# taaha-khan/2023-CompaCT-Image-Compression

Measured on AMD Instinct MI355X. Metric: MPixels/s encode+decode, 12-bit 512x512 CT batch, bytes-exact, higher is better.
Workload: dtype u16

## Files before the change

2023-compact-image-compression_amd/csrc/api.cpp:

```cpp
#include <dlfcn.h>
#include <unistd.h>
#include <zlib.h>

#include <atomic>
#include <chrono>
#include <condition_variable>
#include <functional>
#include <cstdarg>
#include <cstdio>
#include <cstdlib>
#include <cstring>
#include <map>
#include <mutex>
#include <string>
#include <thread>
#include <vector>

#include "../../include/compact_hip.h"
#include "cct_internal.h"
#include "host.h"

namespace cct {
bool gilbert_table(int width, int height, int32_t *out);

// ... 31 lines not shown
	std::mutex *mu = nullptr;
	hipStream_t stream = nullptr;
	struct ZGraph { std::vector<uint8_t> key; hipGraph_t graph = nullptr; hipGraphExec_t exec = nullptr; uint64_t last_use = 0; };
	std::vector<ZGraph> z_graphs;
	uint64_t z_clock = 0;
	hipStream_t stream_copy = nullptr;
	hipEvent_t ev_pack[2] = {nullptr, nullptr}, ev_copied[2] = {nullptr, nullptr};
	DevBuf z_packed2[2];
	unsigned pack_slot = 0;
	DevBuf e_role, e_lidx, e_lmask, e_lcur, e_images, e_payload, e_sizes, e_status, e_stats;
	DevBuf e_pairrec, e_hand;
	DevBuf h_stage;
	DevBuf h_small[2];
	DevBuf z_vals_in, z_vals_out, z_mr, z_rec, z_exitp, z_exitc, z_sym, z_bentry, z_bsym,
	    z_small, z_bend, z_meta, z_tables, z_sorttmp, z_out, z_outsizes, z_in, z_insizes, z_packed, z_packoffs, z_gen, z_runs;
	const void *z_mr_cleared = nullptr;
	size_t z_mr_cleared_cap = 0;
	unsigned z_gen_passes = 0;
	hipEvent_t ev_k0s[2] = {nullptr, nullptr}, ev_k1s[2] = {nullptr, nullptr};
	hipEvent_t ev_z0s[2] = {nullptr, nullptr}, ev_z1s[2] = {nullptr, nullptr};
	hipEvent_t ev_small[2] = {nullptr, nullptr};
	hipStream_t stream_side = nullptr;
	hipEvent_t ev_fork[4] = {nullptr, nullptr, nullptr, nullptr};
	unsigned call_parity = 0;
	DevBuf *all_bufs[48];
	int n_bufs = 0;
	EncSlot()
	{
		DevBuf *b[] = {&e_role, &e_lidx, &e_lmask, &e_lcur, &e_images, &e_payload, &e_sizes, &e_status, &e_stats, &e_pairrec,
		               &e_hand, &h_stage, &z_vals_in, &z_vals_out, &z_mr, &z_rec, &z_exitp, &z_exitc,
		               &z_sym, &z_bentry, &z_bsym, &z_small, &z_bend, &z_meta, &z_tables, &z_sorttmp, &z_out, &z_outsizes, &z_in,
		               &z_insizes, &z_packed, &z_packoffs, &z_packed2[0], &z_packed2[1], &z_gen, &z_runs, &h_small[0], &h_small[1]};
// ... 549 lines not shown
		ta.e = a;
		ta.tile_org = tb->d_org; ta.tile_orient = tb->d_orient; ta.patterns = tb->d_pat;
		ta.n_orient = tb->n_orient; ta.n_tiles = tb->n_tiles; ta.row_pitch = width;
		HIP_TRY(launch_encode_tiles(ta, n, st));
		g_ctx.last_path = 2;
		return CCT_OK;
	}
	const bool run_time = bs_run_time(bs, g_ctx.runtime_bs != 0);
	HIP_TRY(launch_encode(a, n, bs, g_ctx.wg_threads, st, run_time));
	g_ctx.last_path = run_time ? 4 : 0;
	return CCT_OK;
}

constexpr size_t DEFLATE_PASS_BYTES = (size_t)1 << 30;

int deflate_locked(EncSlot &E, const uint8_t *d_in, size_t in_stride, const uint32_t *d_in_sizes, int n, const uint8_t header13[13],
                   size_t out_stride, int level, int strategy)
{
	if (in_stride % 256 != 0 || out_stride % 4 != 0) return fail(CCT_E_ARG, "deflate strides must be multiples of 256 / 4");
	DeflateArgs a{};
	if (!deflate_strategy_args(level, strategy, a))
		return fail(CCT_E_ARG, "zlib level %d with strategy %d is not on the device", level, strategy);
	const bool chains = strategy != 2 && strategy != 3, walk = strategy != 2;
	const size_t EB = (size_t)n * in_stride;
	if (EB >= ((size_t)1 << 32)) return fail(CCT_E_ARG, "deflate batch of %zu bytes exceeds the 4 GiB sort limit; split the batch", EB);
	const int max_blocks = (int)(in_stride / 16383 + 2);
	int rc;
	if (chains) {
		if ((rc = E.z_vals_in.ensure(EB * 8))) return rc;
		if ((rc = E.z_vals_out.ensure(EB * 8))) return rc;
// ... 3 lines not shown
	}
	if ((rc = E.z_sym.ensure(EB * 4))) return rc;
	if (walk) {
		if ((rc = E.z_exitp.ensure(EB * 4))) return rc;
		if ((rc = E.z_exitc.ensure(EB * 4))) return rc;
		if ((rc = E.z_bentry.ensure(EB / 64 * 4))) return rc;
		if ((rc = E.z_bsym.ensure(EB / 64 * 4))) return rc;
	}
	const int run_chunks = (int)(in_stride / 1784 + 1);
	if ((rc = E.z_small.ensure((size_t)n * (9 + 384 + 2 * (size_t)run_chunks) * 4))) return rc;
	if ((rc = E.z_bend.ensure((size_t)n * max_blocks * 4))) return rc;
	if ((rc = E.z_meta.ensure((size_t)n * max_blocks * sizeof(BlockMeta)))) return rc;
	if ((rc = E.z_tables.ensure((size_t)n * max_blocks * sizeof(BlockTables)))) return rc;
	if ((rc = E.z_out.ensure((size_t)n * out_stride))) return rc;
	if ((rc = E.z_outsizes.ensure((size_t)n * 4))) return rc;
	const size_t tmp = (deflate_sort_temp_bytes((size_t)n * in_stride, n) + 511) & ~(size_t)255;
	if ((rc = E.z_sorttmp.ensure(tmp + 256))) return rc;
	const bool use_fork = g_ctx.deflate_fork != 0;
	if (use_fork && !E.stream_side) {
		const int crc = exclusive_section([&]() -> int { HIP_TRY(hipStreamCreateWithFlags(&E.stream_side, hipStreamNonBlocking)); return CCT_OK; });
		if (crc) return crc;
	}
	a.in = d_in; a.in_stride = in_stride; a.in_sizes = d_in_sizes;
	a.rec_in = (uint64_t *)E.z_vals_in.p; a.rec_out = (uint64_t *)E.z_vals_out.p;
	a.pos_mask = (g_ctx.compact_recs && in_stride < ((size_t)1 << 22)) ? (1u << 22) - 1u : 0xFFFFFFFFu;
	uint32_t *small = (uint32_t *)E.z_small.p;
	a.seg_begin = small; a.seg_end = small + n; a.total_syms = small + 2 * n; a.postloop_lit = small + 3 * n;
	a.n_blocks = small + 4 * n; a.adler = small + 5 * n; a.heavy_count = small + 6 * n; a.deep_count = small + 7 * n; a.run_end_count = small + 8 * n; a.sort_hist = small + 9 * n;
	a.run_counts = small + (9 + 384) * (size_t)n; a.run_chunks = run_chunks;
	if ((rc = E.z_gen.ensure(256))) return rc;
	if (chains && (E.z_mr_cleared != E.z_mr.p || E.z_mr_cleared_cap != E.z_mr.cap || E.z_gen_passes >= 16000u)) {
		HIP_TRY(hipMemsetAsync(E.z_mr.p, 0, E.z_mr.cap, E.stream));
		HIP_TRY(hipMemsetAsync(E.z_gen.p, 0, 256, E.stream));
		E.z_mr_cleared = E.z_mr.p; E.z_mr_cleared_cap = E.z_mr.cap; E.z_gen_passes = 0;
	}
	if (chains) E.z_gen_passes++;
	a.gen = (uint32_t *)E.z_gen.p;
	a.mr = E.z_mr.p; a.heavy_list = (uint32_t *)E.z_rec.p; a.sym = (uint32_t *)E.z_sym.p;
	a.run_ends = (uint32_t *)E.z_runs.p;
	a.run_len = (uint16_t *)E.z_sym.p;
	a.rec32 = (uint32_t *)E.z_exitp.p; a.exit_pos = (uint32_t *)E.z_exitc.p; a.exit_cnt = (uint32_t *)E.z_rec.p;
	a.blk_entry = (uint32_t *)E.z_bentry.p; a.blk_symbase = (uint32_t *)E.z_bsym.p;
	a.blk_end = (uint32_t *)E.z_bend.p;
	a.block_meta = (BlockMeta *)E.z_meta.p; a.block_tables = (BlockTables *)E.z_tables.p;
	a.max_blocks = max_blocks;
	a.out = (uint8_t *)E.z_out.p; a.out_stride = out_stride; a.out_sizes = (uint32_t *)E.z_outsizes.p;
	memcpy(a.header13, header13, 13);
	if (g_ctx.use_graph) {
		std::vector<uint8_t> key(sizeof(DeflateArgs) + 2 * sizeof(int));
		memcpy(key.data(), &a, sizeof(DeflateArgs));
		memcpy(key.data() + sizeof(DeflateArgs), &n, sizeof(int));
		const int fork_key = use_fork ? 1 : 0;
		memcpy(key.data() + sizeof(DeflateArgs) + sizeof(int), &fork_key, sizeof(int));
		EncSlot::ZGraph *zg = nullptr;
		for (auto &g : E.z_graphs) if (g.key == key) zg = &g;
		if (!zg) {
			const int crc = exclusive_section([&]() -> int {
				if (E.z_graphs.size() >= 4) {
					size_t old = 0;
					for (size_t i = 1; i < E.z_graphs.size(); i++) if (E.z_graphs[i].last_use < E.z_graphs[old].last_use) old = i;
					if (E.z_graphs[old].exec) (void)hipGraphExecDestroy(E.z_graphs[old].exec);
					if (E.z_graphs[old].graph) (void)hipGraphDestroy(E.z_graphs[old].graph);
					E.z_graphs.erase(E.z_graphs.begin() + (long)old);
				}
				EncSlot::ZGraph g;
				HIP_TRY(hipStreamBeginCapture(E.stream, hipStreamCaptureModeThreadLocal));
				hipError_t le = launch_deflate(a, n, E.z_sorttmp.p, tmp, E.stream, use_fork ? E.stream_side : nullptr, E.ev_fork);
				hipError_t ce = hipStreamEndCapture(E.stream, &g.graph);
				if (le != hipSuccess) { if (g.graph) (void)hipGraphDestroy(g.graph); return fail(CCT_E_DEVICE, "DEFLATE capture: %s", hipGetErrorString(le)); }
				HIP_TRY(ce);
				const hipError_t ie = hipGraphInstantiate(&g.exec, g.graph, nullptr, nullptr, 0);
				if (ie != hipSuccess) { (void)hipGraphDestroy(g.graph); return fail(CCT_E_DEVICE, "hipGraphInstantiate failed: %s", hipGetErrorString(ie)); }
				g.key = key;
				E.z_graphs.push_back(std::move(g));
				return CCT_OK;
			});
			if (crc) return crc;
			zg = &E.z_graphs.back();
		}
		zg->last_use = ++E.z_clock;
		HIP_TRY(hipGraphLaunch(zg->exec, E.stream));
		return CCT_OK;
	}
	HIP_TRY(launch_deflate(a, n, E.z_sorttmp.p, tmp, E.stream, use_fork ? E.stream_side : nullptr, E.ev_fork));
	return CCT_OK;
}

int decode_payload_locked(DecSlot &D, const uint8_t *d_payload, size_t stride, const uint32_t *d_sizes, int n, int width,
                          int height, int bs, int fractal, uint16_t *d_images, uint32_t *d_status, hipStream_t st)
{
	const int N = width * height, NB = N / bs;
	if (stride % 16 != 0) return fail(CCT_E_ARG, "payload stride must be a multiple of 16");
	if (n == 0) return CCT_OK;
	DecArgs a{};
	a.payload = d_payload; a.stride = stride; a.sizes = d_sizes;
	a.lut = nullptr;
	a.n_tiles = 0; a.n_orient = 0; a.width = width;
	if (fractal) {
		const ShapeTables *tb;
// ... 565 lines not shown
				int e = -1; unsigned slot = 0;
				void release() { if (e >= 0) { { std::lock_guard<std::mutex> pl(g_pack_mu); g_pack_busy[e][slot] = false; } g_pack_cv.notify_all(); e = -1; } }
				~PackOwner() { release(); }
			} pack_owner;
			const bool queue_ahead = qa;
			if (queue_ahead) {
				HIP_TRY(hipEventRecord(E.ev_small[par], E.stream));
				{ std::lock_guard<std::mutex> pl(g_pack_mu); g_pack_busy[&E - g_enc][packed_slot] = true; }
				pack_owner.e = (int)(&E - g_enc); pack_owner.slot = (unsigned)packed_slot;
				lk.unlock();
				HIP_TRY(hipEventSynchronize(E.ev_small[par]));
				memcpy(psz.data(), l_psz, (size_t)n * 4); memcpy(h_status, l_status, (size_t)n * 4); memcpy(osz, l_osz, (size_t)nc * 4);
				if (h_stats) memcpy(h_stats, l_stats, (size_t)n * sizeof(cct_slice_stats));
			} else HIP_TRY(hipStreamSynchronize(E.stream));
			drain.disarm();
			HIP_TRY(hipEventElapsedTime(&t_dev_deflate_ms, ev_z0, ev_z1));
			if (one_pass) {
				HIP_TRY(hipEventElapsedTime(&tl_enc_kernel_ms, ev_k0, ev_k1));
				for (int i = 0; i < n; i++)
					if (h_status[i] & CCT_ST_CAP) return fail(CCT_E_CAP, "slice %d overflowed its payload stride", i);
			}
			tl_deflate_ms += t_dev_deflate_ms;
			const double t_c0 = now_ms();
			FilesOut f{E, nc, osz, zstride, 0, std::vector<size_t>(nc + 1, 0)};
			for (int i = 0; i < nc; i++) { f.exact += osz[i]; f.offs[i + 1] = f.offs[i] + (((size_t)osz[i] + 15) & ~(size_t)15); }
			if (packed_slot < 0 && (rc = E.z_packoffs.ensure((size_t)(nc + 1) * 8))) return rc;
			if (!packed) {
				if ((rc = files_to_strided(f, h_out + (size_t)c0 * out_stride, out_stride))) return rc;
				tl_d2h_ms += (float)(now_ms() - t_c0);
				continue;
// ... 85 lines not shown
	HIP_TRY(hipMemcpyAsync(E.z_insizes.p, isz.data(), (size_t)n * 4, hipMemcpyHostToDevice, E.stream));
	uint8_t hdr13[13] = {0};
	struct Events {
		hipEvent_t e[2] = {nullptr, nullptr};
		~Events() { for (hipEvent_t x : e) if (x) (void)hipEventDestroy(x); }
	} ev;
	HIP_TRY(hipEventCreate(&ev.e[0]));
	HIP_TRY(hipEventCreate(&ev.e[1]));
	HIP_TRY(hipEventRecord(ev.e[0], E.stream));
	rc = deflate_locked(E, (const uint8_t *)E.z_in.p, in_stride, (const uint32_t *)E.z_insizes.p, n, hdr13, zstride, level, strategy);
	if (rc) return rc;
	HIP_TRY(hipEventRecord(ev.e[1], E.stream));
	HIP_TRY(hipMemcpyAsync(osz.data(), E.z_outsizes.p, (size_t)n * 4, hipMemcpyDeviceToHost, E.stream));
	HIP_TRY(hipStreamSynchronize(E.stream));
	HIP_TRY(hipEventElapsedTime(&tl_deflate_ms, ev.e[0], ev.e[1]));
	for (int i = 0; i < n; i++) {
		h_out_sizes[i] = osz[i] - 13;
		HIP_TRY(hipMemcpyAsync(h_out + (size_t)i * out_stride, (uint8_t *)E.z_out.p + (size_t)i * zstride + 13, osz[i] - 13,
		                       hipMemcpyDeviceToHost, E.stream));
	}
	HIP_TRY(hipStreamSynchronize(E.stream));
	return CCT_OK;
}

int cct_zlib_compress_batch(const uint8_t *h_in, const uint64_t *h_offsets, int n, uint8_t *h_out, size_t out_stride,
                            uint32_t *h_out_sizes)
{
	return zlib_compress_batch_impl(h_in, h_offsets, n, 9, Z_DEFAULT_STRATEGY, h_out, out_stride, h_out_sizes);
}

// ... 326 lines not shown
```

2023-compact-image-compression_amd/csrc/cct_internal.h:

```cpp
#pragma once
#include <stddef.h>
#include <stdint.h>

#include <hip/hip_runtime.h>

namespace cct {

constexpr int ENC_CH = 8192;
constexpr int ENC_RING = 4;
constexpr int ENC_LIST_CAP = 1536;
constexpr int ENC_STG_BYTES = 2 * ENC_CH + ENC_CH / 8 + 64;
constexpr int ENC_MAX_LDS_ROLE = 48 * 1024;

constexpr uint8_t ROLE_PARTNER = 0xFF;

struct EncArgs {
	const uint16_t *images;
	const int32_t *lut;
	int N, NB;
	int eof;
	uint32_t flags;
	uint8_t *payload; size_t stride;
	uint32_t *sizes; uint32_t *status;
	uint8_t *ws_role;
// ... 92 lines not shown
struct BlockTables {
	uint16_t lcode[286]; uint8_t llen[286];
	uint16_t dcode[30]; uint8_t dlen[30];
	uint32_t hdr_bits[160];
};
struct DeflateArgs {
	const uint8_t *in; size_t in_stride; const uint32_t *in_sizes;
	uint64_t *rec_in, *rec_out;
	uint32_t pos_mask;
	uint32_t *seg_begin, *seg_end;
	void *mr;
	uint32_t *gen;
	uint32_t *heavy_list, *sym, *run_ends;
	uint32_t *run_counts; int run_chunks;
	uint32_t *sort_hist;
	uint16_t *run_len;
	uint32_t *rec32, *exit_pos, *exit_cnt;
	uint32_t *blk_entry, *blk_symbase;
	uint32_t *total_syms, *postloop_lit, *n_blocks, *adler, *heavy_count, *deep_count, *run_end_count;
	uint32_t *blk_end;
	BlockMeta *block_meta; BlockTables *block_tables;
	int max_blocks;
	uint8_t *out; size_t out_stride; uint32_t *out_sizes;
	uint8_t header13[16];
	uint32_t good, max_lazy, nice, max_chain, zlib_flg;
	uint32_t strategy, min_len;
};
bool deflate_level_args(int level, DeflateArgs &a);
bool deflate_strategy_args(int level, int strategy, DeflateArgs &a);
hipError_t deflate_init_tables();
size_t deflate_sort_temp_bytes(size_t total, int n);
hipError_t launch_pack(const uint8_t *src, size_t stride, const uint32_t *sizes, int n, uint64_t *offsets, uint8_t *dst,
                       int exact, hipStream_t st);
hipError_t launch_deflate(const DeflateArgs &a, int n, void *sort_temp, size_t sort_temp_bytes, hipStream_t st, hipStream_t side = nullptr,
                          const hipEvent_t *fork_join_events = nullptr);

hipError_t launch_gate_bump(uint32_t *word, hipStream_t st);
hipError_t launch_gate_wait(const uint32_t *gate, uint32_t want_pass, uint32_t grace_us, uint32_t timeout_us, hipStream_t st);

struct InflateArgs {
	const uint8_t *in; uint64_t in_total;
	const uint64_t *offsets; int skip;
	uint8_t *out; size_t out_stride;
	uint32_t *out_sizes, *status;
};
hipError_t launch_inflate(const InflateArgs &a, int n, hipStream_t st, int lanes);

hipError_t launch_packbits_encode(const uint8_t *d_in, const uint64_t *d_offsets, int n, int delta, uint32_t *d_ws, uint8_t *d_out,
                                  size_t out_stride, uint32_t *d_out_sizes, hipStream_t st);
// ... 5 lines not shown
```

2023-compact-image-compression_amd/csrc/deflate_kernels.hip:

```cpp
#include <hip/hip_runtime.h>
#include <cstring>
#include <algorithm>

#include "cct_internal.h"
#include "../../include/compact_hip.h"

namespace cct {
namespace {

constexpr int MIN_MATCH = 3, MAX_MATCH = 258, WSIZE = 32768;
constexpr int MIN_LOOKAHEAD = MAX_MATCH + MIN_MATCH + 1;
constexpr int MAX_DIST = WSIZE - MIN_LOOKAHEAD;
constexpr int TOO_FAR = 4096;
constexpr int BLOCK_SYMS = 16383;
constexpr int L_CODES = 286, D_CODES = 30, BL_CODES = 19, HEAP_SIZE = 2 * L_CODES + 1;
constexpr int END_BLOCK = 256, MAX_BITS = 15, MAX_BL_BITS = 7;
constexpr uint32_t Z_FILTERED = 1, Z_HUFFMAN_ONLY = 2, Z_RLE = 3, Z_FIXED = 4;
__host__ __device__ __forceinline__ bool short_pass(uint32_t strategy) { return strategy == Z_HUFFMAN_ONLY || strategy == Z_RLE; }

__constant__ uint8_t c_extra_lbits[29] = {0,0,0,0,0,0,0,0,1,1,1,1,2,2,2,2,3,3,3,3,4,4,4,4,5,5,5,5,0};
__constant__ uint8_t c_extra_dbits[30] = {0,0,0,0,1,1,2,2,3,3,4,4,5,5,6,6,7,7,8,8,9,9,10,10,11,11,12,12,13,13};
__constant__ uint8_t c_extra_blbits[19] = {0,0,0,0,0,0,0,0,0,0,0,0,0,0,0,0,2,3,7};
__constant__ uint8_t c_bl_order[19] = {16,17,18,0,8,7,9,6,10,5,11,4,12,3,13,2,14,1,15};
__constant__ uint8_t c_length_code[256];
// ... 27 lines not shown
	return o;
}

__device__ __forceinline__ void lds_barrier()
{
	asm volatile("s_waitcnt lgkmcnt(0)\n\ts_barrier" ::: "memory");
}

__device__ __forceinline__ uint32_t wave_sum(uint32_t v)
{
#pragma unroll
	for (int d = 32; d >= 1; d >>= 1) v += (uint32_t)__shfl_xor((int)v, d, 64);
	return v;
}

template <bool FIRST>
__global__ void __launch_bounds__(1024) dfl_sort_pass_kernel(DeflateArgs a)
{
	constexpr int BITS = FIRST ? 8 : 7, NB = 1 << BITS;
	__shared__ uint32_t offs[256];
	__shared__ uint32_t wcnt[16][NB];
	const int s = blockIdx.x;
	const uint32_t L = a.in_sizes[s];
	const uint8_t *in = a.in + (size_t)s * a.in_stride;
	const size_t base = (size_t)s * a.in_stride;
	const uint32_t npos = L >= MIN_MATCH ? L - 2 : 0;
	const uint64_t *rec_src = a.rec_in + base;
	uint64_t *rec_dst = (FIRST ? a.rec_in : a.rec_out) + base;
	const int tid = threadIdx.x, lane = tid & 63, wave = tid >> 6;
	const uint64_t lt_mask = (1ull << lane) - 1ull;
	if (tid < 256) offs[tid] = 0;
	__syncthreads();
	if (tid < NB) offs[tid] = a.sort_hist[(size_t)s * 384 + (FIRST ? 0 : 256) + tid];
	__syncthreads();
	if (wave == 0) {
		uint32_t v[4], sum = 0;
#pragma unroll
		for (int k = 0; k < 4; k++) { v[k] = offs[lane * 4 + k]; sum += v[k]; }
		uint32_t inc = sum;
#pragma unroll
		for (int d = 1; d < 64; d <<= 1) { const uint32_t o = (uint32_t)__shfl_up((int)inc, d, 64); if (lane >= d) inc += o; }
		uint32_t run = inc - sum;
#pragma unroll
		for (int k = 0; k < 4; k++) { offs[lane * 4 + k] = run; run += v[k]; }
	}
	__syncthreads();
#ifndef CCT_SORT_E
#define CCT_SORT_E 4
#endif
	constexpr int E = CCT_SORT_E;
	constexpr int ND = E / 4;
	const uint32_t last = npos ? npos - 1 : 0;
	static_assert(E % 4 == 0 && ND + 1 <= E, "pass A: whole dwords per lane, kept in ra[0 .. ND]");
#ifdef CCT_SORT_PROBE
	const bool compact = false;
#else
	const bool compact = a.pos_mask != 0xFFFFFFFFu;
#endif
	const uint32_t dmax = (uint32_t)a.in_stride - 4u;
	auto fetch = [&](uint32_t tile_base, uint32_t (&ra)[E], uint32_t (&rb)[E]) {
		if (FIRST) {
#pragma unroll
			for (int d = 0; d < ND; d++) ra[d] = *reinterpret_cast<const uint32_t *>(in + min(tile_base + 256u * d + 4u * (uint32_t)lane, dmax));
			ra[ND] = *reinterpret_cast<const uint32_t *>(in + min(tile_base + 256u * ND, dmax));
#pragma unroll
			for (int e = 0; e < E; e++) rb[e] = compact ? a.run_len[base + min(tile_base + (uint32_t)(e * 64 + lane), last)] : 0u;
		} else {
#pragma unroll
			for (int e = 0; e < E; e++) {
				const uint64_t r = rec_src[min(tile_base + (uint32_t)(e * 64 + lane), last)];
				ra[e] = (uint32_t)r; rb[e] = (uint32_t)(r >> 32);
			}
		}
	};
	auto finish = [&](uint32_t tile_base, const uint32_t (&ra)[E], const uint32_t (&rb)[E], uint32_t (&h)[E], uint32_t (&p)[E]) {
#pragma unroll
		for (int e = 0; e < E; e++) {
			const uint32_t idx = tile_base + (uint32_t)(e * 64 + lane);
			if (FIRST) {
				const int la = (e & 3) * 16 + (lane >> 2);
				const uint32_t da = (uint32_t)__builtin_amdgcn_ds_bpermute(la << 2, (int)ra[e >> 2]);
				uint32_t db = (uint32_t)__builtin_amdgcn_ds_bpermute(((la + 1) & 63) << 2, (int)ra[e >> 2]);
				if ((e & 3) == 3) {
					const uint32_t nxt = (e >> 2) + 1 < ND ? (uint32_t)__builtin_amdgcn_readfirstlane((int)ra[(e >> 2) + 1 < ND ? (e >> 2) + 1 : 0]) : ra[ND];
					if (la == 63) db = nxt;
				}
				const uint32_t sh = (uint32_t)lane & 3u;
				const uint32_t w = __builtin_amdgcn_alignbyte(db, da, sh);
				const uint32_t b0 = w & 255u, b1 = (w >> 8) & 255u, b2 = (w >> 16) & 255u;
				h[e] = ((b0 << 10) ^ (b1 << 5) ^ b2) & 0x7FFFu; p[e] = idx;
				if (compact) {
					const uint32_t b4 = (db >> (8u * sh)) & 255u;
					const uint32_t f16 = (b0 == b1 && b1 == b2) ? rb[e] : ((w >> 24) | (b4 << 8));
					h[e] |= (f16 << 15) | ((b0 >> 7) << 31); p[e] |= (b1 << 22) | (((b0 >> 5) & 3u) << 30);
				}
			}
			else { h[e] = rb[e]; p[e] = ra[e]; }
			if (idx >= npos) { h[e] = 0; p[e] = idx; }
		}
	};
	uint32_t hn[E], pn[E];
	{
		uint32_t ra[E], rb[E];
		fetch((uint32_t)(wave * 64 * E), ra, rb);
		finish((uint32_t)(wave * 64 * E), ra, rb, hn, pn);
	}
	for (uint32_t t0 = 0; t0 < npos; t0 += 1024 * E) {
		uint32_t h[E], p[E], rk[E], ra[E], rb[E];
		const uint32_t idx0 = t0 + (uint32_t)(wave * 64 * E + lane);
#pragma unroll
		for (int e = 0; e < E; e++) { h[e] = hn[e]; p[e] = pn[e]; }
		const uint32_t next_base = t0 + (uint32_t)(1024 * E + wave * 64 * E);
		fetch(next_base, ra, rb);
		for (int k = lane; k < NB; k += 64) wcnt[wave][k] = 0;
#pragma unroll
		for (int e = 0; e < E; e++) {
			const bool valid = idx0 + e * 64 < npos;
			const uint32_t d = FIRST ? (h[e] & 255u) : ((h[e] & 0x7FFFu) >> 8);
			uint64_t same = __ballot(valid);
#pragma unroll
			for (int b = 0; b < BITS; b++) {
				const bool bit = (d >> b) & 1u;
				const uint64_t bal = __ballot(bit);
				same &= bit ? bal : ~bal;
			}
			const uint32_t rank = (uint32_t)__popcll(same & lt_mask);
			uint32_t before = 0;
			if (valid) {
				before = wcnt[wave][d];
				if (rank == 0) wcnt[wave][d] = before + (uint32_t)__popcll(same);
			}
			rk[e] = before + rank;
		}
		lds_barrier();
		if (tid < NB) {
			uint32_t c[16], run = offs[tid];
#pragma unroll
			for (int w = 0; w < 16; w++) c[w] = wcnt[w][tid];
#pragma unroll
			for (int w = 0; w < 16; w++) { wcnt[w][tid] = run; run += c[w]; }
			offs[tid] = run;
		}
		lds_barrier();
#pragma unroll
		for (int e = 0; e < E; e++) asm volatile("" : "+v"(ra[e]), "+v"(rb[e]) :: "memory");
		finish(next_base, ra, rb, hn, pn);
#pragma unroll
		for (int e = 0; e < E; e++) {
			if (idx0 + e * 64 < npos) {
				const uint32_t d = FIRST ? (h[e] & 255u) : ((h[e] & 0x7FFFu) >> 8);
				const uint32_t dst = wcnt[wave][d] + rk[e];
				rec_dst[dst] = (uint64_t)p[e] | ((uint64_t)h[e] << 32);
			}
		}
	}
}

constexpr int LIGHT_STEPS = 12;

__device__ __forceinline__ bool xcd_slice(int n, int &s, uint32_t &part, uint32_t &nparts)
{
	const uint32_t lin = blockIdx.x + gridDim.x * blockIdx.y;
	const uint32_t c = lin & 7u, k = lin >> 3;
	nparts = gridDim.x;
	s = (int)(8u * (k / nparts) + c);
	part = k % nparts;
	return s < n;
}

// ... 1378 lines not shown
		BlockMeta bm = meta[m];
		bm.bit_off = bit;
		if (bm.type == 0) {
			bit = (bit + 3 + 7) & ~7ull;
			bit += 32 + 8ull * bm.stored_len;
		} else {
			bit += 3 + bm.hdr_nbits + bm.body_bits;
		}
		if (bm.last) bit = (bit + 7) & ~7ull;
		meta[m] = bm;
	}
	const uint64_t byte = bit >> 3;
	const uint32_t ad = a.adler[s];
	out[byte + 0] = (uint8_t)(ad >> 24); out[byte + 1] = (uint8_t)(ad >> 16);
	out[byte + 2] = (uint8_t)(ad >> 8);  out[byte + 3] = (uint8_t)ad;
	a.out_sizes[s] = (uint32_t)(byte + 4);
}

__device__ __forceinline__ void or_bits(uint32_t *words, uint64_t bit, uint64_t value, int nbits)
{
	if (nbits == 0) return;
	const uint64_t w = bit >> 5;
	const int sh = (int)(bit & 31);
	const uint64_t lo = value << sh;
	const uint64_t hi = sh ? (value >> (64 - sh)) : 0ull;
	atomicOr(&words[w], (uint32_t)lo);
	if (sh + nbits > 32) atomicOr(&words[w + 1], (uint32_t)(lo >> 32));
	if (sh + nbits > 64) atomicOr(&words[w + 2], (uint32_t)hi);
}

__global__ void __launch_bounds__(256) dfl_emit_kernel(DeflateArgs a)
// ... 139 lines not shown
	for (uint32_t i = blockIdx.x * blockDim.x + threadIdx.x; i < n16; i += gridDim.x * blockDim.x) out[i] = in[i];
}

__global__ void dfl_offsets2_kernel(DeflateArgs a, int n)
{
	const size_t per = a.in_stride / 64;
	for (size_t i = blockIdx.x * (size_t)blockDim.x + threadIdx.x; i < (size_t)n * per; i += (size_t)gridDim.x * blockDim.x)
		a.blk_entry[i] = 0xFFFFFFFFu;
}

__global__ void dfl_offsets_kernel(DeflateArgs a, int n)
{
	if (blockIdx.x == 0) {
		for (int s = threadIdx.x; s < n; s += blockDim.x) { a.postloop_lit[s] = 0; a.heavy_count[s] = 0; a.deep_count[s] = 0; a.run_end_count[s] = 0; }
		if (threadIdx.x == 0) *a.gen = *a.gen % GEN_MAX + 1u;
	}
	const size_t nrc = (size_t)n * 2 * (size_t)a.run_chunks;
	for (size_t t = (size_t)blockIdx.x * blockDim.x + threadIdx.x; t < nrc; t += (size_t)gridDim.x * blockDim.x) a.run_counts[t] = 0;
}

}

bool deflate_level_args(int level, DeflateArgs &a)
{
	static const uint32_t T[6][5] = {
		{4, 4, 16, 16, 0x5E}, {8, 16, 32, 32, 0x5E}, {8, 16, 128, 128, 0x9C},
		{8, 32, 128, 256, 0xDA}, {32, 128, 258, 1024, 0xDA}, {32, 258, 258, 4096, 0xDA},
	};
	if (level < 4 || level > 9) return false;
	const uint32_t *t = T[level - 4];
// ... 49 lines not shown
	for (int bits = 1; bits <= 15; bits++) { c = (c + bl_count[bits - 1]) << 1; next_code[bits] = (uint16_t)c; }
	auto rev = [](unsigned v, int len) { unsigned r = 0; do { r |= v & 1; v >>= 1; r <<= 1; } while (--len > 0); return r >> 1; };
	for (n = 0; n < 288; n++) static_lcode[n] = (uint16_t)rev(next_code[static_llen[n]]++, static_llen[n]);
	for (n = 0; n < 30; n++) static_dcode[n] = (uint16_t)rev((unsigned)n, 5);
	hipError_t e;
	if ((e = hipMemcpyToSymbol(HIP_SYMBOL(c_length_code), length_code, sizeof length_code)) != hipSuccess) return e;
	if ((e = hipMemcpyToSymbol(HIP_SYMBOL(c_base_length), base_length, sizeof base_length)) != hipSuccess) return e;
	if ((e = hipMemcpyToSymbol(HIP_SYMBOL(c_dist_code), dist_code, sizeof dist_code)) != hipSuccess) return e;
	if ((e = hipMemcpyToSymbol(HIP_SYMBOL(c_base_dist), base_dist, sizeof base_dist)) != hipSuccess) return e;
	if ((e = hipMemcpyToSymbol(HIP_SYMBOL(c_static_lcode), static_lcode, sizeof static_lcode)) != hipSuccess) return e;
	if ((e = hipMemcpyToSymbol(HIP_SYMBOL(c_static_llen), static_llen, sizeof static_llen)) != hipSuccess) return e;
	if ((e = hipMemcpyToSymbol(HIP_SYMBOL(c_static_dcode), static_dcode, sizeof static_dcode)) != hipSuccess) return e;
	return hipSuccess;
}

size_t deflate_sort_temp_bytes(size_t total, int n)
{
	(void)total; (void)n;
	return 0;
}

static hipError_t launch_deflate_short(const DeflateArgs &a, int n, hipStream_t st)
{
	const int gx = (int)std::min<size_t>(64, (a.in_stride + 255) / 256);
	if (a.strategy == Z_RLE) {
		hipLaunchKernelGGL(dfl_run_len_kernel<false>, dim3(gx, n), dim3(256), 0, st, a);
		hipLaunchKernelGGL(dfl_rle_rec_kernel, dim3(gx, n), dim3(256), 0, st, a);
		hipLaunchKernelGGL(dfl_offsets2_kernel, dim3(256), dim3(256), 0, st, a, n);
		hipLaunchKernelGGL(dfl_walk_kernel, dim3(n), dim3(WALK_T), 0, st, a, n);
		hipLaunchKernelGGL(dfl_symbols_kernel, dim3(gx, n), dim3(256), 0, st, a);
	} else {
		hipLaunchKernelGGL(dfl_huff_symbols_kernel, dim3(gx, n), dim3(256), 0, st, a);
	}
	hipLaunchKernelGGL(dfl_adler_kernel, dim3(n), dim3(256), 0, st, a);
	hipLaunchKernelGGL(dfl_tree_kernel, dim3((a.max_blocks + TREE_BLOCKS - 1) / TREE_BLOCKS, n), dim3(64), 0, st, a);
	hipLaunchKernelGGL(dfl_layout_kernel, dim3((n + 63) / 64), dim3(64), 0, st, a, n);
	hipLaunchKernelGGL(dfl_emit_kernel, dim3(a.max_blocks, n), dim3(256), 0, st, a);
	return hipGetLastError();
}

hipError_t launch_deflate(const DeflateArgs &a, int n, void *sort_temp, size_t sort_temp_bytes, hipStream_t st, hipStream_t side,
                          const hipEvent_t *ev)
{
	hipError_t e;
	if ((e = hipMemsetAsync(a.out, 0, (size_t)n * a.out_stride, st)) != hipSuccess) return e;
	if (short_pass(a.strategy)) return launch_deflate_short(a, n, st);
	if ((e = hipMemsetAsync(a.sort_hist, 0, (size_t)n * 384 * 4, st)) != hipSuccess) return e;
	hipLaunchKernelGGL(dfl_offsets_kernel, dim3(64), dim3(256), 0, st, a, n);
	const int gx = (int)std::min<size_t>(64, (a.in_stride + 255) / 256);
	(void)sort_temp; (void)sort_temp_bytes;
	hipLaunchKernelGGL(dfl_run_len_kernel<true>, dim3(gx, n), dim3(256), 0, st, a);
	hipLaunchKernelGGL(dfl_sort_pass_kernel<true>, dim3(n), dim3(1024), 0, st, a);
	hipLaunchKernelGGL(dfl_sort_pass_kernel<false>, dim3(n), dim3(1024), 0, st, a);
	const bool fork = side != nullptr && ev != nullptr;
	hipStream_t s2 = fork ? side : st;
	if (fork) {
		if ((e = hipEventRecord(ev[0], st)) != hipSuccess) return e;
		if ((e = hipStreamWaitEvent(s2, ev[0], 0)) != hipSuccess) return e;
	}
	hipLaunchKernelGGL(dfl_run_lists_kernel, dim3(a.run_chunks, n), dim3(256), 0, s2, a);
	hipLaunchKernelGGL(dfl_run_info_kernel, dim3(8, n), dim3(256), 0, s2, a);
	const int gm_cap = a.pos_mask == COMPACT_POS_MASK ? 256 : 2048;
	const int gm = (int)std::min<size_t>(gm_cap, (a.in_stride + 255) / 256), n8 = (n + 7) & ~7;
	if (a.max_chain < 16 || a.max_chain > 4096 || a.nice < 16 || a.nice > (uint32_t)MAX_MATCH) return hipErrorInvalidValue;
	const bool ql = (a.max_chain >> 2) <= (uint32_t)LIGHT_STEPS;
	if (a.pos_mask == COMPACT_POS_MASK) {
		if (ql) hipLaunchKernelGGL((dfl_match_kernel<true, true>), dim3(gm, n8), dim3(256), 0, st, a, n);
		else hipLaunchKernelGGL((dfl_match_kernel<true, false>), dim3(gm, n8), dim3(256), 0, st, a, n);
	} else if (a.pos_mask == 0xFFFFFFFFu) {
		if (ql) hipLaunchKernelGGL((dfl_match_kernel<false, true>), dim3(gm, n8), dim3(256), 0, st, a, n);
		else hipLaunchKernelGGL((dfl_match_kernel<false, false>), dim3(gm, n8), dim3(256), 0, st, a, n);
	} else return hipErrorInvalidValue;
	if (fork) {
		if ((e = hipEventRecord(ev[1], st)) != hipSuccess) return e;
		if ((e = hipEventRecord(ev[2], s2)) != hipSuccess) return e;
		if ((e = hipStreamWaitEvent(s2, ev[1], 0)) != hipSuccess) return e;
		if ((e = hipStreamWaitEvent(st, ev[2], 0)) != hipSuccess) return e;
	}
// ... 38 lines not shown
```

Before: 16360.

## Split DEFLATE radix sort passes into tiles with decoupled look-back scan

Replaces the one-workgroup-per-slice radix sort passes with a multi-tile kernel where each workgroup sorts a tile and obtains its per-digit offsets through a decoupled look-back over status words in device memory. The aim is to spread each slice's sort across many workgroups instead of serializing it inside one 1024-thread block. It adds a status buffer that is cleared only when reallocated, generation tags, dynamic tile ordering via atomic counters, and a timeout path that marks output sizes as zero. A host-side check then reports an error for those slices. The risks are spin-wait cost and correctness hazards in the cross-workgroup protocol.

Result: no change. 16420, median of 6 (+0.4%).

```diff
diff --git a/2023-compact-image-compression_amd/csrc/api.cpp b/2023-compact-image-compression_amd/csrc/api.cpp
--- a/2023-compact-image-compression_amd/csrc/api.cpp
+++ b/2023-compact-image-compression_amd/csrc/api.cpp
@@ -69,8 +69,8 @@
 	DevBuf h_small[2];
 	DevBuf z_vals_in, z_vals_out, z_mr, z_rec, z_exitp, z_exitc, z_sym, z_bentry, z_bsym,
 	    z_small, z_bend, z_meta, z_tables, z_sorttmp, z_out, z_outsizes, z_in, z_insizes, z_packed, z_packoffs, z_gen, z_runs;
-	const void *z_mr_cleared = nullptr;
-	size_t z_mr_cleared_cap = 0;
+	const void *z_mr_cleared = nullptr, *z_sort_cleared = nullptr;
+	size_t z_mr_cleared_cap = 0, z_sort_cleared_cap = 0;
 	unsigned z_gen_passes = 0;
 	hipEvent_t ev_k0s[2] = {nullptr, nullptr}, ev_k1s[2] = {nullptr, nullptr};
 	hipEvent_t ev_z0s[2] = {nullptr, nullptr}, ev_z1s[2] = {nullptr, nullptr};
@@ -650,6 +650,13 @@
 
 constexpr size_t DEFLATE_PASS_BYTES = (size_t)1 << 30;
 
+static int check_deflate_sizes(const uint32_t *osz, int n)
+{
+	for (int i = 0; i < n; i++)
+		if (!osz[i]) return fail(CCT_E_DEVICE, "device DEFLATE: a sort tile waited 1 s for the tiles before it; the pass was abandoned");
+	return CCT_OK;
+}
+
 int deflate_locked(EncSlot &E, const uint8_t *d_in, size_t in_stride, const uint32_t *d_in_sizes, int n, const uint8_t header13[13],
                    size_t out_stride, int level, int strategy)
 {
@@ -683,8 +690,7 @@
 	if ((rc = E.z_tables.ensure((size_t)n * max_blocks * sizeof(BlockTables)))) return rc;
 	if ((rc = E.z_out.ensure((size_t)n * out_stride))) return rc;
 	if ((rc = E.z_outsizes.ensure((size_t)n * 4))) return rc;
-	const size_t tmp = (deflate_sort_temp_bytes((size_t)n * in_stride, n) + 511) & ~(size_t)255;
-	if ((rc = E.z_sorttmp.ensure(tmp + 256))) return rc;
+	if (chains && (rc = E.z_sorttmp.ensure(deflate_sort_temp_bytes(in_stride, n)))) return rc;
 	const bool use_fork = g_ctx.deflate_fork != 0;
 	if (use_fork && !E.stream_side) {
 		const int crc = exclusive_section([&]() -> int { HIP_TRY(hipStreamCreateWithFlags(&E.stream_side, hipStreamNonBlocking)); return CCT_OK; });
@@ -700,11 +706,22 @@
 	if ((rc = E.z_gen.ensure(256))) return rc;
 	if (chains && (E.z_mr_cleared != E.z_mr.p || E.z_mr_cleared_cap != E.z_mr.cap || E.z_gen_passes >= 16000u)) {
 		HIP_TRY(hipMemsetAsync(E.z_mr.p, 0, E.z_mr.cap, E.stream));
+		HIP_TRY(hipMemsetAsync(E.z_sorttmp.p, 0, E.z_sorttmp.cap, E.stream));
 		HIP_TRY(hipMemsetAsync(E.z_gen.p, 0, 256, E.stream));
 		E.z_mr_cleared = E.z_mr.p; E.z_mr_cleared_cap = E.z_mr.cap; E.z_gen_passes = 0;
+		E.z_sort_cleared = E.z_sorttmp.p; E.z_sort_cleared_cap = E.z_sorttmp.cap;
+	}
+	if (chains && (E.z_sort_cleared != E.z_sorttmp.p || E.z_sort_cleared_cap != E.z_sorttmp.cap)) {
+		HIP_TRY(hipMemsetAsync(E.z_sorttmp.p, 0, E.z_sorttmp.cap, E.stream));
+		E.z_sort_cleared = E.z_sorttmp.p; E.z_sort_cleared_cap = E.z_sorttmp.cap;
 	}
 	if (chains) E.z_gen_passes++;
 	a.gen = (uint32_t *)E.z_gen.p;
+	if (chains) {
+		a.sort_tiles = deflate_sort_tiles(in_stride);
+		a.sort_status = (uint64_t *)E.z_sorttmp.p;
+		a.sort_ctl = (uint32_t *)(a.sort_status + (size_t)n * a.sort_tiles * 256);
+	}
 	a.mr = E.z_mr.p; a.heavy_list = (uint32_t *)E.z_rec.p; a.sym = (uint32_t *)E.z_sym.p;
 	a.run_ends = (uint32_t *)E.z_runs.p;
 	a.run_len = (uint16_t *)E.z_sym.p;
@@ -734,7 +751,7 @@
 				}
 				EncSlot::ZGraph g;
 				HIP_TRY(hipStreamBeginCapture(E.stream, hipStreamCaptureModeThreadLocal));
-				hipError_t le = launch_deflate(a, n, E.z_sorttmp.p, tmp, E.stream, use_fork ? E.stream_side : nullptr, E.ev_fork);
+				hipError_t le = launch_deflate(a, n, E.stream, use_fork ? E.stream_side : nullptr, E.ev_fork);
 				hipError_t ce = hipStreamEndCapture(E.stream, &g.graph);
 				if (le != hipSuccess) { if (g.graph) (void)hipGraphDestroy(g.graph); return fail(CCT_E_DEVICE, "DEFLATE capture: %s", hipGetErrorString(le)); }
 				HIP_TRY(ce);
@@ -751,7 +768,7 @@
 		HIP_TRY(hipGraphLaunch(zg->exec, E.stream));
 		return CCT_OK;
 	}
-	HIP_TRY(launch_deflate(a, n, E.z_sorttmp.p, tmp, E.stream, use_fork ? E.stream_side : nullptr, E.ev_fork));
+	HIP_TRY(launch_deflate(a, n, E.stream, use_fork ? E.stream_side : nullptr, E.ev_fork));
 	return CCT_OK;
 }
 
@@ -1347,6 +1364,7 @@
 				if (h_stats) memcpy(h_stats, l_stats, (size_t)n * sizeof(cct_slice_stats));
 			} else HIP_TRY(hipStreamSynchronize(E.stream));
 			drain.disarm();
+			if ((rc = check_deflate_sizes(osz, nc))) return rc;
 			HIP_TRY(hipEventElapsedTime(&t_dev_deflate_ms, ev_z0, ev_z1));
 			if (one_pass) {
 				HIP_TRY(hipEventElapsedTime(&tl_enc_kernel_ms, ev_k0, ev_k1));
@@ -1462,6 +1480,7 @@
 	HIP_TRY(hipMemcpyAsync(osz.data(), E.z_outsizes.p, (size_t)n * 4, hipMemcpyDeviceToHost, E.stream));
 	HIP_TRY(hipStreamSynchronize(E.stream));
 	HIP_TRY(hipEventElapsedTime(&tl_deflate_ms, ev.e[0], ev.e[1]));
+	if ((rc = check_deflate_sizes(osz.data(), n))) return rc;
 	for (int i = 0; i < n; i++) {
 		h_out_sizes[i] = osz[i] - 13;
 		HIP_TRY(hipMemcpyAsync(h_out + (size_t)i * out_stride, (uint8_t *)E.z_out.p + (size_t)i * zstride + 13, osz[i] - 13,
diff --git a/2023-compact-image-compression_amd/csrc/cct_internal.h b/2023-compact-image-compression_amd/csrc/cct_internal.h
--- a/2023-compact-image-compression_amd/csrc/cct_internal.h
+++ b/2023-compact-image-compression_amd/csrc/cct_internal.h
@@ -130,6 +130,8 @@
 	uint32_t *heavy_list, *sym, *run_ends;
 	uint32_t *run_counts; int run_chunks;
 	uint32_t *sort_hist;
+	uint64_t *sort_status; int sort_tiles;
+	uint32_t *sort_ctl;
 	uint16_t *run_len;
 	uint32_t *rec32, *exit_pos, *exit_cnt;
 	uint32_t *blk_entry, *blk_symbase;
@@ -145,10 +147,11 @@
 bool deflate_level_args(int level, DeflateArgs &a);
 bool deflate_strategy_args(int level, int strategy, DeflateArgs &a);
 hipError_t deflate_init_tables();
-size_t deflate_sort_temp_bytes(size_t total, int n);
+int deflate_sort_tiles(size_t in_stride);
+size_t deflate_sort_temp_bytes(size_t in_stride, int n);
 hipError_t launch_pack(const uint8_t *src, size_t stride, const uint32_t *sizes, int n, uint64_t *offsets, uint8_t *dst,
                        int exact, hipStream_t st);
-hipError_t launch_deflate(const DeflateArgs &a, int n, void *sort_temp, size_t sort_temp_bytes, hipStream_t st, hipStream_t side = nullptr,
+hipError_t launch_deflate(const DeflateArgs &a, int n, hipStream_t st, hipStream_t side = nullptr,
                           const hipEvent_t *fork_join_events = nullptr);
 
 hipError_t launch_gate_bump(uint32_t *word, hipStream_t st);
diff --git a/2023-compact-image-compression_amd/csrc/deflate_kernels.hip b/2023-compact-image-compression_amd/csrc/deflate_kernels.hip
--- a/2023-compact-image-compression_amd/csrc/deflate_kernels.hip
+++ b/2023-compact-image-compression_amd/csrc/deflate_kernels.hip
@@ -65,109 +65,142 @@
 	return v;
 }
 
+#ifndef CCT_SORT_WAVES
+#define CCT_SORT_WAVES 8
+#endif
+#ifndef CCT_SORT_E
+#define CCT_SORT_E 8
+#endif
+constexpr int SORT_WAVES = CCT_SORT_WAVES, SORT_E = CCT_SORT_E;
+constexpr int SORT_T = 64 * SORT_WAVES, SORT_TILE = SORT_T * SORT_E;
+static_assert(SORT_T >= 256 && SORT_T <= 1024, "one lane per digit in the look-back");
+static_assert(SORT_E % 4 == 0, "pass A: whole dwords per lane");
+
+constexpr uint32_t SORT_AGG = 1, SORT_INC = 2;
+constexpr int SORT_LOOKBACK = 4;
+constexpr uint64_t SORT_SPIN_TICKS = 100000000ull;
+__device__ __forceinline__ uint64_t sort_word(uint32_t flag, uint32_t tag, uint32_t count)
+{
+	return (uint64_t)count | ((uint64_t)flag << 32) | ((uint64_t)tag << 34);
+}
+
+__device__ __forceinline__ bool sort_lookback(uint64_t *st, uint32_t tile, uint32_t tag, uint32_t count, uint32_t &excl, uint32_t *err)
+{
+	__hip_atomic_store(st + (size_t)tile * 256, sort_word(SORT_AGG, tag, count), __ATOMIC_RELAXED, __HIP_MEMORY_SCOPE_AGENT);
+	uint32_t sum = 0;
+	int j = (int)tile - 1;
+	uint64_t t_stall = 0;
+	bool ok = true;
+	for (;;) {
+		uint64_t w[SORT_LOOKBACK];
+#pragma unroll
+		for (int k = 0; k < SORT_LOOKBACK; k++)
+			w[k] = __hip_atomic_load(st + (size_t)max(j - k, 0) * 256, __ATOMIC_RELAXED, __HIP_MEMORY_SCOPE_AGENT);
+		uint32_t add = 0;
+		int adv = 0;
+		bool inc = false, stall = false;
+#pragma unroll
+		for (int k = 0; k < SORT_LOOKBACK; k++) {
+			const uint32_t f = (uint32_t)(w[k] >> 34) == tag ? (uint32_t)(w[k] >> 32) & 3u : 0u;
+			if (!inc && !stall) {
+				if (f) { add += (uint32_t)w[k]; adv++; inc = f == SORT_INC; }
+				else stall = true;
+			}
+		}
+		sum += add; j -= adv;
+		if (inc) break;
+		if (stall) {
+			const uint64_t now = wall_clock64();
+			if (adv || !t_stall) t_stall = now;
+			else if (now - t_stall > SORT_SPIN_TICKS) { ok = false; atomicOr(err, 1u); break; }
+			__builtin_amdgcn_s_sleep(1);
+		}
+	}
+	excl = sum;
+	__hip_atomic_store(st + (size_t)tile * 256, sort_word(SORT_INC, tag, sum + count), __ATOMIC_RELAXED, __HIP_MEMORY_SCOPE_AGENT);
+	return ok;
+}
+
 template <bool FIRST>
-__global__ void __launch_bounds__(1024) dfl_sort_pass_kernel(DeflateArgs a)
-{
-	constexpr int BITS = FIRST ? 8 : 7, NB = 1 << BITS;
-	__shared__ uint32_t offs[256];
-	__shared__ uint32_t wcnt[16][NB];
-	const int s = blockIdx.x;
+__global__ void __launch_bounds__(SORT_T) dfl_sort_tile_kernel(DeflateArgs a, int n)
+{
+	constexpr int BITS = FIRST ? 8 : 7, NB = 1 << BITS, E = SORT_E, ND = E / 4;
+	__shared__ uint32_t wcnt[SORT_WAVES][NB];
+	__shared__ uint32_t sh_tile, sh_fail, sh_wsum[4];
+	const uint32_t lin = blockIdx.x + gridDim.x * blockIdx.y;
+	const int s = (int)(8u * ((lin >> 3) % (gridDim.y >> 3)) + (lin & 7u));
+	if (s >= n) return;
+	const int tid = threadIdx.x, lane = tid & 63, wave = tid >> 6;
+	if (tid == 0) { sh_tile = atomicAdd(a.sort_ctl + 2 * s + (FIRST ? 0 : 1), 1u); sh_fail = 0; }
+	__syncthreads();
+	const uint32_t tile = sh_tile;
 	const uint32_t L = a.in_sizes[s];
+	const uint32_t npos = L >= MIN_MATCH ? L - 2 : 0;
+	if (tile >= (npos + SORT_TILE - 1) / SORT_TILE) return;
 	const uint8_t *in = a.in + (size_t)s * a.in_stride;
 	const size_t base = (size_t)s * a.in_stride;
-	const uint32_t npos = L >= MIN_MATCH ? L - 2 : 0;
 	const uint64_t *rec_src = a.rec_in + base;
 	uint64_t *rec_dst = (FIRST ? a.rec_in : a.rec_out) + base;
-	const int tid = threadIdx.x, lane = tid & 63, wave = tid >> 6;
 	const uint64_t lt_mask = (1ull << lane) - 1ull;
-	if (tid < 256) offs[tid] = 0;
-	__syncthreads();
-	if (tid < NB) offs[tid] = a.sort_hist[(size_t)s * 384 + (FIRST ? 0 : 256) + tid];
-	__syncthreads();
-	if (wave == 0) {
-		uint32_t v[4], sum = 0;
-#pragma unroll
-		for (int k = 0; k < 4; k++) { v[k] = offs[lane * 4 + k]; sum += v[k]; }
-		uint32_t inc = sum;
+	const uint32_t last = npos - 1;
+	const uint32_t wb = tile * (uint32_t)SORT_TILE + (uint32_t)(wave * 64 * E);
+	const bool compact = a.pos_mask != 0xFFFFFFFFu;
+	uint32_t ra[E], rb[E];
+	if (FIRST) {
+		const uint32_t dmax = (uint32_t)a.in_stride - 4u;
+#pragma unroll
+		for (int d = 0; d < ND; d++) ra[d] = *reinterpret_cast<const uint32_t *>(in + min(wb + 256u * d + 4u * (uint32_t)lane, dmax));
+		ra[ND] = *reinterpret_cast<const uint32_t *>(in + min(wb + 256u * ND, dmax));
+#pragma unroll
+		for (int e = 0; e < E; e++) rb[e] = compact ? a.run_len[base + min(wb + (uint32_t)(e * 64 + lane), last)] : 0u;
+	} else {
+#pragma unroll
+		for (int e = 0; e < E; e++) {
+			const uint64_t r = rec_src[min(wb + (uint32_t)(e * 64 + lane), last)];
+			ra[e] = (uint32_t)r; rb[e] = (uint32_t)(r >> 32);
+		}
+	}
+	for (int k = lane; k < NB; k += 64) wcnt[wave][k] = 0;
+	uint32_t bucket = 0;
+	if (tile == 0) {
+		const uint32_t v = tid < NB ? a.sort_hist[(size_t)s * 384 + (FIRST ? 0 : 256) + tid] : 0u;
+		uint32_t inc = v;
 #pragma unroll
 		for (int d = 1; d < 64; d <<= 1) { const uint32_t o = (uint32_t)__shfl_up((int)inc, d, 64); if (lane >= d) inc += o; }
-		uint32_t run = inc - sum;
-#pragma unroll
-		for (int k = 0; k < 4; k++) { offs[lane * 4 + k] = run; run += v[k]; }
-	}
-	__syncthreads();
-#ifndef CCT_SORT_E
-#define CCT_SORT_E 4
-#endif
-	constexpr int E = CCT_SORT_E;
-	constexpr int ND = E / 4;
-	const uint32_t last = npos ? npos - 1 : 0;
-	static_assert(E % 4 == 0 && ND + 1 <= E, "pass A: whole dwords per lane, kept in ra[0 .. ND]");
-#ifdef CCT_SORT_PROBE
-	const bool compact = false;
-#else
-	const bool compact = a.pos_mask != 0xFFFFFFFFu;
-#endif
-	const uint32_t dmax = (uint32_t)a.in_stride - 4u;
-	auto fetch = [&](uint32_t tile_base, uint32_t (&ra)[E], uint32_t (&rb)[E]) {
+		if (lane == 63 && wave < 4) sh_wsum[wave] = inc;
+		lds_barrier();
+		bucket = inc - v;
+		for (int w = 0; w < wave && w < 4; w++) bucket += sh_wsum[w];
+	}
+	uint32_t h[E], p[E], rk[E];
+#pragma unroll
+	for (int e = 0; e < E; e++) {
+		const uint32_t idx = wb + (uint32_t)(e * 64 + lane);
 		if (FIRST) {
-#pragma unroll
-			for (int d = 0; d < ND; d++) ra[d] = *reinterpret_cast<const uint32_t *>(in + min(tile_base + 256u * d + 4u * (uint32_t)lane, dmax));
-			ra[ND] = *reinterpret_cast<const uint32_t *>(in + min(tile_base + 256u * ND, dmax));
-#pragma unroll
-			for (int e = 0; e < E; e++) rb[e] = compact ? a.run_len[base + min(tile_base + (uint32_t)(e * 64 + lane), last)] : 0u;
+			const int la = (e & 3) * 16 + (lane >> 2);
+			const uint32_t da = (uint32_t)__builtin_amdgcn_ds_bpermute(la << 2, (int)ra[e >> 2]);
+			uint32_t db = (uint32_t)__builtin_amdgcn_ds_bpermute(((la + 1) & 63) << 2, (int)ra[e >> 2]);
+			if ((e & 3) == 3) {
+				const uint32_t nxt = (e >> 2) + 1 < ND ? (uint32_t)__builtin_amdgcn_readfirstlane((int)ra[(e >> 2) + 1 < ND ? (e >> 2) + 1 : 0]) : ra[ND];
+				if (la == 63) db = nxt;
+			}
+			const uint32_t sh = (uint32_t)lane & 3u;
+			const uint32_t w = __builtin_amdgcn_alignbyte(db, da, sh);
+			const uint32_t b0 = w & 255u, b1 = (w >> 8) & 255u, b2 = (w >> 16) & 255u;
+			h[e] = ((b0 << 10) ^ (b1 << 5) ^ b2) & 0x7FFFu; p[e] = idx;
+			if (compact) {
+				const uint32_t b4 = (db >> (8u * sh)) & 255u;
+				const uint32_t f16 = (b0 == b1 && b1 == b2) ? rb[e] : ((w >> 24) | (b4 << 8));
+				h[e] |= (f16 << 15) | ((b0 >> 7) << 31); p[e] |= (b1 << 22) | (((b0 >> 5) & 3u) << 30);
+			}
+		}
+		else { h[e] = rb[e]; p[e] = ra[e]; }
+		const bool valid = idx < npos;
+		const uint32_t d = FIRST ? (h[e] & 255u) : ((h[e] & 0x7FFFu) >> 8);
+		uint32_t rank, cnt;
+		if (__all(valid && d == (uint32_t)__builtin_amdgcn_readfirstlane((int)d))) {
+			rank = (uint32_t)lane; cnt = 64;
 		} else {
-#pragma unroll
-			for (int e = 0; e < E; e++) {
-				const uint64_t r = rec_src[min(tile_base + (uint32_t)(e * 64 + lane), last)];
-				ra[e] = (uint32_t)r; rb[e] = (uint32_t)(r >> 32);
-			}
-		}
-	};
-	auto finish = [&](uint32_t tile_base, const uint32_t (&ra)[E], const uint32_t (&rb)[E], uint32_t (&h)[E], uint32_t (&p)[E]) {
-#pragma unroll
-		for (int e = 0; e < E; e++) {
-			const uint32_t idx = tile_base + (uint32_t)(e * 64 + lane);
-			if (FIRST) {
-				const int la = (e & 3) * 16 + (lane >> 2);
-				const uint32_t da = (uint32_t)__builtin_amdgcn_ds_bpermute(la << 2, (int)ra[e >> 2]);
-				uint32_t db = (uint32_t)__builtin_amdgcn_ds_bpermute(((la + 1) & 63) << 2, (int)ra[e >> 2]);
-				if ((e & 3) == 3) {
-					const uint32_t nxt = (e >> 2) + 1 < ND ? (uint32_t)__builtin_amdgcn_readfirstlane((int)ra[(e >> 2) + 1 < ND ? (e >> 2) + 1 : 0]) : ra[ND];
-					if (la == 63) db = nxt;
-				}
-				const uint32_t sh = (uint32_t)lane & 3u;
-				const uint32_t w = __builtin_amdgcn_alignbyte(db, da, sh);
-				const uint32_t b0 = w & 255u, b1 = (w >> 8) & 255u, b2 = (w >> 16) & 255u;
-				h[e] = ((b0 << 10) ^ (b1 << 5) ^ b2) & 0x7FFFu; p[e] = idx;
-				if (compact) {
-					const uint32_t b4 = (db >> (8u * sh)) & 255u;
-					const uint32_t f16 = (b0 == b1 && b1 == b2) ? rb[e] : ((w >> 24) | (b4 << 8));
-					h[e] |= (f16 << 15) | ((b0 >> 7) << 31); p[e] |= (b1 << 22) | (((b0 >> 5) & 3u) << 30);
-				}
-			}
-			else { h[e] = rb[e]; p[e] = ra[e]; }
-			if (idx >= npos) { h[e] = 0; p[e] = idx; }
-		}
-	};
-	uint32_t hn[E], pn[E];
-	{
-		uint32_t ra[E], rb[E];
-		fetch((uint32_t)(wave * 64 * E), ra, rb);
-		finish((uint32_t)(wave * 64 * E), ra, rb, hn, pn);
-	}
-	for (uint32_t t0 = 0; t0 < npos; t0 += 1024 * E) {
-		uint32_t h[E], p[E], rk[E], ra[E], rb[E];
-		const uint32_t idx0 = t0 + (uint32_t)(wave * 64 * E + lane);
-#pragma unroll
-		for (int e = 0; e < E; e++) { h[e] = hn[e]; p[e] = pn[e]; }
-		const uint32_t next_base = t0 + (uint32_t)(1024 * E + wave * 64 * E);
-		fetch(next_base, ra, rb);
-		for (int k = lane; k < NB; k += 64) wcnt[wave][k] = 0;
-#pragma unroll
-		for (int e = 0; e < E; e++) {
-			const bool valid = idx0 + e * 64 < npos;
-			const uint32_t d = FIRST ? (h[e] & 255u) : ((h[e] & 0x7FFFu) >> 8);
 			uint64_t same = __ballot(valid);
 #pragma unroll
 			for (int b = 0; b < BITS; b++) {
@@ -175,35 +208,37 @@
 				const uint64_t bal = __ballot(bit);
 				same &= bit ? bal : ~bal;
 			}
-			const uint32_t rank = (uint32_t)__popcll(same & lt_mask);
-			uint32_t before = 0;
-			if (valid) {
-				before = wcnt[wave][d];
-				if (rank == 0) wcnt[wave][d] = before + (uint32_t)__popcll(same);
-			}
-			rk[e] = before + rank;
-		}
-		lds_barrier();
-		if (tid < NB) {
-			uint32_t c[16], run = offs[tid];
-#pragma unroll
-			for (int w = 0; w < 16; w++) c[w] = wcnt[w][tid];
-#pragma unroll
-			for (int w = 0; w < 16; w++) { wcnt[w][tid] = run; run += c[w]; }
-			offs[tid] = run;
-		}
-		lds_barrier();
-#pragma unroll
-		for (int e = 0; e < E; e++) asm volatile("" : "+v"(ra[e]), "+v"(rb[e]) :: "memory");
-		finish(next_base, ra, rb, hn, pn);
-#pragma unroll
-		for (int e = 0; e < E; e++) {
-			if (idx0 + e * 64 < npos) {
-				const uint32_t d = FIRST ? (h[e] & 255u) : ((h[e] & 0x7FFFu) >> 8);
-				const uint32_t dst = wcnt[wave][d] + rk[e];
-				rec_dst[dst] = (uint64_t)p[e] | ((uint64_t)h[e] << 32);
-			}
-		}
+			rank = (uint32_t)__popcll(same & lt_mask); cnt = (uint32_t)__popcll(same);
+		}
+		uint32_t before = 0;
+		if (valid) {
+			before = wcnt[wave][d];
+			if (rank == 0) wcnt[wave][d] = before + cnt;
+		}
+		rk[e] = before + rank;
+	}
+	lds_barrier();
+	if (tid < NB) {
+		uint32_t c[SORT_WAVES], tot = 0;
+#pragma unroll
+		for (int w = 0; w < SORT_WAVES; w++) c[w] = wcnt[w][tid];
+#pragma unroll
+		for (int w = 0; w < SORT_WAVES; w++) { wcnt[w][tid] = tot; tot += c[w]; }
+		uint64_t *st = a.sort_status + (size_t)s * a.sort_tiles * 256 + tid;
+		const uint32_t tag = 2u * *a.gen + (FIRST ? 0u : 1u);
+		uint32_t start = bucket;
+		if (tile == 0) __hip_atomic_store(st, sort_word(SORT_INC, tag, bucket + tot), __ATOMIC_RELAXED, __HIP_MEMORY_SCOPE_AGENT);
+		else if (!sort_lookback(st, tile, tag, tot, start, a.sort_ctl + 2 * n)) sh_fail = 1;
+#pragma unroll
+		for (int w = 0; w < SORT_WAVES; w++) wcnt[w][tid] += start;
+	}
+	lds_barrier();
+	if (sh_fail) return;
+#pragma unroll
+	for (int e = 0; e < E; e++) {
+		const uint32_t d = FIRST ? (h[e] & 255u) : ((h[e] & 0x7FFFu) >> 8);
+		const uint32_t dst = wcnt[wave][d] + rk[e];
+		if (wb + (uint32_t)(e * 64 + lane) < npos && dst < npos) rec_dst[dst] = (uint64_t)p[e] | ((uint64_t)h[e] << 32);
 	}
 }
 
@@ -1612,7 +1647,7 @@
 	const uint32_t ad = a.adler[s];
 	out[byte + 0] = (uint8_t)(ad >> 24); out[byte + 1] = (uint8_t)(ad >> 16);
 	out[byte + 2] = (uint8_t)(ad >> 8);  out[byte + 3] = (uint8_t)ad;
-	a.out_sizes[s] = (uint32_t)(byte + 4);
+	a.out_sizes[s] = !short_pass(a.strategy) && a.sort_ctl[2 * n] ? 0u : (uint32_t)(byte + 4);
 }
 
 __device__ __forceinline__ void or_bits(uint32_t *words, uint64_t bit, uint64_t value, int nbits)
@@ -1782,6 +1817,7 @@
 	if (blockIdx.x == 0) {
 		for (int s = threadIdx.x; s < n; s += blockDim.x) { a.postloop_lit[s] = 0; a.heavy_count[s] = 0; a.deep_count[s] = 0; a.run_end_count[s] = 0; }
 		if (threadIdx.x == 0) *a.gen = *a.gen % GEN_MAX + 1u;
+		for (int t = threadIdx.x; t <= 2 * n; t += blockDim.x) a.sort_ctl[t] = 0;
 	}
 	const size_t nrc = (size_t)n * 2 * (size_t)a.run_chunks;
 	for (size_t t = (size_t)blockIdx.x * blockDim.x + threadIdx.x; t < nrc; t += (size_t)gridDim.x * blockDim.x) a.run_counts[t] = 0;
@@ -1861,10 +1897,14 @@
 	return hipSuccess;
 }
 
-size_t deflate_sort_temp_bytes(size_t total, int n)
-{
-	(void)total; (void)n;
-	return 0;
+int deflate_sort_tiles(size_t in_stride)
+{
+	return (int)((in_stride + SORT_TILE - 1) / SORT_TILE);
+}
+
+size_t deflate_sort_temp_bytes(size_t in_stride, int n)
+{
+	return (size_t)n * (size_t)deflate_sort_tiles(in_stride) * 256 * 8 + ((size_t)2 * n + 1) * 4;
 }
 
 static hipError_t launch_deflate_short(const DeflateArgs &a, int n, hipStream_t st)
@@ -1886,19 +1926,18 @@
 	return hipGetLastError();
 }
 
-hipError_t launch_deflate(const DeflateArgs &a, int n, void *sort_temp, size_t sort_temp_bytes, hipStream_t st, hipStream_t side,
-                          const hipEvent_t *ev)
+hipError_t launch_deflate(const DeflateArgs &a, int n, hipStream_t st, hipStream_t side, const hipEvent_t *ev)
 {
 	hipError_t e;
 	if ((e = hipMemsetAsync(a.out, 0, (size_t)n * a.out_stride, st)) != hipSuccess) return e;
 	if (short_pass(a.strategy)) return launch_deflate_short(a, n, st);
 	if ((e = hipMemsetAsync(a.sort_hist, 0, (size_t)n * 384 * 4, st)) != hipSuccess) return e;
 	hipLaunchKernelGGL(dfl_offsets_kernel, dim3(64), dim3(256), 0, st, a, n);
-	const int gx = (int)std::min<size_t>(64, (a.in_stride + 255) / 256);
-	(void)sort_temp; (void)sort_temp_bytes;
+	const int gx = (int)std::min<size_t>(64, (a.in_stride + 255) / 256), n8 = (n + 7) & ~7;
+	if (a.sort_tiles != deflate_sort_tiles(a.in_stride)) return hipErrorInvalidValue;
 	hipLaunchKernelGGL(dfl_run_len_kernel<true>, dim3(gx, n), dim3(256), 0, st, a);
-	hipLaunchKernelGGL(dfl_sort_pass_kernel<true>, dim3(n), dim3(1024), 0, st, a);
-	hipLaunchKernelGGL(dfl_sort_pass_kernel<false>, dim3(n), dim3(1024), 0, st, a);
+	hipLaunchKernelGGL(dfl_sort_tile_kernel<true>, dim3(a.sort_tiles, n8), dim3(SORT_T), 0, st, a, n);
+	hipLaunchKernelGGL(dfl_sort_tile_kernel<false>, dim3(a.sort_tiles, n8), dim3(SORT_T), 0, st, a, n);
 	const bool fork = side != nullptr && ev != nullptr;
 	hipStream_t s2 = fork ? side : st;
 	if (fork) {
@@ -1908,7 +1947,7 @@
 	hipLaunchKernelGGL(dfl_run_lists_kernel, dim3(a.run_chunks, n), dim3(256), 0, s2, a);
 	hipLaunchKernelGGL(dfl_run_info_kernel, dim3(8, n), dim3(256), 0, s2, a);
 	const int gm_cap = a.pos_mask == COMPACT_POS_MASK ? 256 : 2048;
-	const int gm = (int)std::min<size_t>(gm_cap, (a.in_stride + 255) / 256), n8 = (n + 7) & ~7;
+	const int gm = (int)std::min<size_t>(gm_cap, (a.in_stride + 255) / 256);
 	if (a.max_chain < 16 || a.max_chain > 4096 || a.nice < 16 || a.nice > (uint32_t)MAX_MATCH) return hipErrorInvalidValue;
 	const bool ql = (a.max_chain >> 2) <= (uint32_t)LIGHT_STEPS;
 	if (a.pos_mask == COMPACT_POS_MASK) {
```
